# ddemidov/amgcl

Hardware: AMD Instinct MI355X
Metric: setup+solve time (s) & iterations to 1e-6, 3D Poisson 512^3 (lower is better)
Workload: dtype fp64; 1 GPU; model=3D Poisson 512^3 (7-point stencil), unknowns=134217728, solver=cg, precond=smoothed_aggregation AMG + SPAI0, iters=16, parallelism=single GPU

## Files before the change

amgcl_amd/backend/_hiplib.py:

```python
import ctypes
import os

_LIB = None

_SIGS = {
    "amg_spmv_f64": [ctypes.c_int64, ctypes.c_int64, ctypes.c_void_p, ctypes.c_void_p,
                     ctypes.c_void_p, ctypes.c_void_p, ctypes.c_double, ctypes.c_double,
                     ctypes.c_void_p, ctypes.c_int, ctypes.c_void_p],
    "amg_residual_f64": [ctypes.c_int64, ctypes.c_int64, ctypes.c_void_p, ctypes.c_void_p,
                         ctypes.c_void_p, ctypes.c_void_p, ctypes.c_void_p, ctypes.c_void_p,
                         ctypes.c_int, ctypes.c_void_p],
    "amg_relax_diag_f64": [ctypes.c_int64, ctypes.c_int64, ctypes.c_void_p, ctypes.c_void_p,
                           ctypes.c_void_p, ctypes.c_void_p, ctypes.c_void_p, ctypes.c_void_p,
                           ctypes.c_void_p, ctypes.c_int, ctypes.c_void_p],
    "amg_axpby_f64": [ctypes.c_int64, ctypes.c_double, ctypes.c_void_p, ctypes.c_double,
                      ctypes.c_void_p, ctypes.c_void_p],
    "amg_axpbypcz_f64": [ctypes.c_int64, ctypes.c_double, ctypes.c_void_p, ctypes.c_double,
                         ctypes.c_void_p, ctypes.c_double, ctypes.c_void_p, ctypes.c_void_p],
    "amg_vmul_f64": [ctypes.c_int64, ctypes.c_double, ctypes.c_void_p, ctypes.c_void_p,
                     ctypes.c_double, ctypes.c_void_p, ctypes.c_void_p],
    "amg_fill_f64": [ctypes.c_int64, ctypes.c_double, ctypes.c_void_p, ctypes.c_void_p],
    "amg_dot_f64": [ctypes.c_int64, ctypes.c_void_p, ctypes.c_void_p, ctypes.c_void_p,
                    ctypes.c_void_p],
    "amg_dot2_f64": [ctypes.c_int64, ctypes.c_void_p, ctypes.c_void_p, ctypes.c_void_p,
# ... 72 lines not shown
    "amg_sort_rows": [ctypes.c_int64] + [ctypes.c_void_p] * 4,
    "amg_spgemm_count": [ctypes.c_int64] + [ctypes.c_void_p] * 9,
    "amg_spgemm_fill": [ctypes.c_int64] + [ctypes.c_void_p] * 10 + [ctypes.c_int]
                       + [ctypes.c_void_p] * 2,
    "amg_gershgorin": [ctypes.c_int64, ctypes.c_void_p, ctypes.c_void_p, ctypes.c_void_p, ctypes.c_int, ctypes.c_void_p, ctypes.c_void_p],
    "amg_poisson_cnt": [ctypes.c_int64] * 4 + [ctypes.c_void_p] * 2,
    "amg_poisson_fill": [ctypes.c_int64] * 4 + [ctypes.c_void_p] * 4,
}

for _op in ("spmv", "residual", "relax_diag", "axpby", "axpbypcz", "vmul", "fill", "dot",
            "gather", "scatter", "gemv", "sell_spmv", "sell_residual", "sell_relax",
            "sell_fill"):
    _SIGS[f"amg_{_op}_f32"] = _SIGS[f"amg_{_op}_f64"]


def lib():
    global _LIB
    if _LIB is None:
        path = os.path.join(os.path.dirname(os.path.dirname(os.path.abspath(__file__))),
                            "_hip", "libamghip.so")
        if not os.path.exists(path):
            from ..build import build_hip_lib

            build_hip_lib()
        if not os.path.exists(path):
            raise RuntimeError(
                f"libamghip.so not found at {path}; run `python setup.py build_ext "
                "--inplace` — GPU ops do not fall back to eager torch"
            )
        _LIB = ctypes.CDLL(path)
        for name, argtypes in _SIGS.items():
            fn = getattr(_LIB, name)
            fn.argtypes = argtypes
            fn.restype = ctypes.c_int
    return _LIB


def check(rc, what):
    if rc != 0:
        raise RuntimeError(f"HIP kernel '{what}' failed with hipError_t={rc}")
```

amgcl_amd/csrc/hip/amg_common.h:

```cpp
#pragma once
#include <hip/hip_runtime.h>
#include <cstdint>

#define WAVE 64

__device__ static inline int64_t amg_logical_block() {
#ifdef AMGCL_SWIZZLE
    unsigned g = gridDim.x;
    if ((g & 7u) == 0u)
        return (int64_t)(blockIdx.x & 7u) * (int64_t)(g >> 3) + (blockIdx.x >> 3);
#endif
    return blockIdx.x;
}

#ifdef AMGCL_NT
#define AMG_STREAM_LD(p) __builtin_nontemporal_load(p)
#else
#define AMG_STREAM_LD(p) (*(p))
#endif

static inline int amg_nblocks(int64_t work, int block = 256, int cap = 2048) {
    int64_t b = (work + block - 1) / block;
    if (b < 1) b = 1;
    if (b > cap) b = cap;
    if (b > 8) b = (b + 7) & ~(int64_t)7;
    return (int)b;
}

static inline int amg_pick_subw(int64_t nrows, int64_t nnz) {
    double m = nrows ? (double)nnz / (double)nrows : 1.0;
    if (m <= 4) return 2;
    if (m <= 10) return 4;
    if (m <= 24) return 8;
    if (m <= 128) return 16;
// ... 45 lines not shown
```

amgcl_amd/csrc/hip/amg_kernels.h:

```cpp
#pragma once
#include <hip/hip_runtime.h>
#include <cstdint>

struct OpDesc;
struct LevelDesc;

extern "C" {

int amg_spmv_f64(int64_t nrows, int64_t nnz, const int *ptr, const int *col,
                 const double *val, const double *x, double alpha, double beta,
                 double *y, int subw, hipStream_t stream);
int amg_spmv_f32(int64_t nrows, int64_t nnz, const int *ptr, const int *col,
                 const float *val, const float *x, double alpha, double beta, float *y,
                 int subw, hipStream_t stream);
int amg_residual_f64(int64_t nrows, int64_t nnz, const int *ptr, const int *col,
                     const double *val, const double *rhs, const double *x, double *r,
                     int subw, hipStream_t stream);
int amg_residual_f32(int64_t nrows, int64_t nnz, const int *ptr, const int *col,
                     const float *val, const float *rhs, const float *x, float *r,
                     int subw, hipStream_t stream);
int amg_sell_spmv_f64(int64_t nrows, int64_t nslice, const int64_t *soff, const int *col,
                      const double *val, const int *srows, const double *x, double alpha,
                      double beta, double *y, hipStream_t stream);
int amg_sell_spmv_f32(int64_t nrows, int64_t nslice, const int64_t *soff, const int *col,
// ... 26 lines not shown
int amg_vmul_f64(int64_t n, double a, const double *m, const double *x, double b,
                 double *z, hipStream_t stream);
int amg_vmul_f32(int64_t n, double a, const float *m, const float *x, double b, float *z,
                 hipStream_t stream);
int amg_fill_f64(int64_t n, double v, double *x, hipStream_t stream);
int amg_fill_f32(int64_t n, double v, float *x, hipStream_t stream);
int amg_dot_f64(int64_t n, const double *x, const double *y, double *out,
                hipStream_t stream);
int amg_dot2_f64(int64_t n, const double *x1, const double *y1, const double *x2,
                 const double *y2, double *out, hipStream_t stream);
int amg_gemv_f64(int64_t n, const double *a, const double *f, double *u,
                 hipStream_t stream);
int amg_gemv_f32(int64_t n, const float *a, const float *f, float *u, hipStream_t stream);
int amg_cg_tail_f64(int64_t n, double alpha, const double *p, const double *q, double *x,
                    double *r, double *out, hipStream_t stream);
int amg_cast_d2s(int64_t n, const double *src, float *dst, hipStream_t stream);
int amg_cast_s2d(int64_t n, const float *src, double *dst, hipStream_t stream);

int amg_bsr_spmv_f64(int64_t nbrows, int bsize, const int *ptr, const int *col,
                     const double *val, const double *x, double alpha, double beta,
                     double *y, hipStream_t stream);
int amg_bsr_residual_f64(int64_t nbrows, int bsize, const int *ptr, const int *col,
                         const double *val, const double *rhs, const double *x,
                         double *r, hipStream_t stream);
int amg_bsr_relax_f64(int64_t nbrows, int bsize, const int *ptr, const int *col,
                      const double *val, const double *M, const double *rhs,
                      const double *x, double *t, hipStream_t stream);

int amg_setup_diag(int64_t n, const int *ptr, const int *col, const double *val,
                   double *d, hipStream_t s);
// ... 16 lines not shown
int amg_transpose_count(int64_t nnz, const int *col, int *tcnt, hipStream_t s);
int amg_transpose_scatter(int64_t n, const int *ptr, const int *col, const double *val,
                          int *cursor, int *tcol, double *tval, hipStream_t s);
int amg_spgemm_count(int64_t an, const int *aptr, const int *acol, const int *bptr,
                     const int *bcol, int *ub, int *cnt, int *overflow, int *bigscratch,
                     hipStream_t s);
int amg_spgemm_fill(int64_t an, const int *aptr, const int *acol, const double *aval,
                    const int *bptr, const int *bcol, const double *bval, const int *ub,
                    const int *cptr_scanned, int *ccol, double *cval, int do_sort,
                    const int *bigscratch, hipStream_t s);

void *amg_driver_create(const LevelDesc *levels, int nlevels, const void *coarse_inv,
                        int64_t ncoarse, int npre, int npost, int ncycle, int pre_cycles,
                        int f32, const OpDesc *a64, hipStream_t stream);
void amg_driver_destroy(void *h);
int amg_driver_precond(void *h, const double *rhs, double *x, double *x_swap);
int amg_driver_cg(void *h, const double *rhs, double *x, double *r, double *s, double *p,
                  double *q, double *s_swap, double tol, double abstol, int maxiter,
                  int64_t *iters_out, double *resid_out);
int amg_driver_bicgstab(void *h, const double *rhs, double *x, double *r, double *p,
                        double *v, double *s2, double *t2, double *rh, double *T,
                        double *T_swap, double tol, double abstol, int maxiter,
                        int64_t *iters_out, double *resid_out);

}
```

amgcl_amd/csrc/hip/driver.hip:

```cpp

#include <hip/hip_runtime.h>

#include "amg_common.h"
#include "amg_kernels.h"

#include <cmath>
#include <cstddef>
#include <cstdint>
#include <cstdlib>
#include <type_traits>
#include <utility>
#include <vector>

#define AMG_BY_TYPE(name)                                 \
    template <typename T, typename... Args>               \
    static inline int name(Args... args) {                \
        if constexpr (std::is_same_v<T, double>)          \
            return amg_##name##_f64(args...);             \
        else                                              \
            return amg_##name##_f32(args...);             \
    }
AMG_BY_TYPE(spmv)
AMG_BY_TYPE(residual)
AMG_BY_TYPE(gemv)
AMG_BY_TYPE(sell_spmv)
AMG_BY_TYPE(sell_residual)
AMG_BY_TYPE(sell_relax)
AMG_BY_TYPE(axpby)
AMG_BY_TYPE(vmul)
AMG_BY_TYPE(fill)
#undef AMG_BY_TYPE

template <int SUBW, typename T>
__global__ void relax_swap_k(int64_t nrows, const int *__restrict__ ptr,
                             const int *__restrict__ col, const T *__restrict__ val,
                             const T *__restrict__ M, const T *__restrict__ rhs,
                             const T *__restrict__ x, T *__restrict__ xn) {
    int64_t tid = amg_logical_block() * blockDim.x + threadIdx.x;
    int lane = (int)(tid & (SUBW - 1));
    int64_t row = tid / SUBW;
    int64_t stride = ((int64_t)gridDim.x * blockDim.x) / SUBW;
    for (; row < nrows; row += stride) {
        T s = (T)0;
        int b = ptr[row], e = ptr[row + 1];
        for (int j = b + lane; j < e; j += SUBW)
            s += AMG_STREAM_LD(&val[j]) * x[AMG_STREAM_LD(&col[j])];
#pragma unroll
        for (int off = SUBW / 2; off > 0; off >>= 1) s += __shfl_down(s, off, SUBW);
        if (lane == 0) xn[row] = x[row] + M[row] * (rhs[row] - s);
    }
}

template <typename T>
__global__ void relax_zero_k(int64_t n, const T *__restrict__ M,
                             const T *__restrict__ rhs, T *__restrict__ xn) {
    int64_t i = (int64_t)blockIdx.x * blockDim.x + threadIdx.x;
    int64_t stride = (int64_t)gridDim.x * blockDim.x;
    for (; i < n; i += stride) xn[i] = M[i] * rhs[i];
}

struct GraphEntry {
    const double *rhs;
    double *x;
    double *xswap;
    hipGraphExec_t exec;
};

struct Driver {
    std::vector<LevelDesc> lv;
    const void *coarse_inv;
    int64_t ncoarse;
    int npre, npost, ncycle, pre_cycles;
    hipStream_t stream;
    double *dotbuf_d;
    double *dotbuf_h;
    std::vector<GraphEntry> graphs;
    bool use_graphs;
    hipStream_t ext_stream;
    hipEvent_t ev_in, ev_out;
    int f32;
    OpDesc a64;
    float *cb_r, *cb_x, *cb_s;
};

#define CHK(x)                          \
    do {                                \
        int _rc = (x);                  \
        if (_rc) return _rc;            \
    } while (0)

template <typename T>
static int op_spmv(Driver *D, const OpDesc &op, const T *x, double alpha, double beta,
                   T *y) {
    if (op.nslice)
        return sell_spmv<T>(op.nrows, op.nslice, op.soff, op.scol, (const T *)op.sval,
                            op.srows, x, alpha, beta, y, D->stream);
    return spmv<T>(op.nrows, op.nnz, op.ptr, op.col, (const T *)op.val, x, alpha, beta, y,
                   op.subw, D->stream);
// ... 57 lines not shown
        CHK(amg_axpby_f64(n, 1.0, t, 1.0, s, st));
        CHK(amg_axpby_f64(n, om, s, 1.0 - om, y, st));
    }
    CHK(hipMemcpyAsync(b, y, n * sizeof(double), hipMemcpyDeviceToDevice, st));
    CHK(amg_vmul_f64(n, 1.0, L.ilu_dinv, b, 0.0, y, st));
    for (int it = 0; it < L.ilu_iters; ++it) {
        CHK(op_spmv<double>(D, L.ilu_U, y, -1.0, 0.0, s));
        CHK(amg_axpby_f64(n, 1.0, b, 1.0, s, st));
        CHK(amg_vmul_f64(n, 1.0, L.ilu_dinv, s, 0.0, s, st));
        CHK(amg_axpby_f64(n, om, s, 1.0 - om, y, st));
    }
    CHK(amg_axpby_f64(n, L.ilu_damping, y, 1.0, x, st));
    return 0;
}

template <typename T>
static int relax_swap(Driver *D, const LevelDesc &L, const T *rhs, T **x, T **xn) {
    if (L.ilu_iters) {
        CHK(ilu_apply<T>(D, L, rhs, *x, *xn));
        return 0;
    }
    if (L.cheb_degree) {
        CHK(cheb_apply<T>(D, L, rhs, *x, *xn));
        return 0;
    }
    if (L.bsize) {
        if constexpr (std::is_same_v<T, double>)
            CHK(amg_bsr_relax_f64(L.nbrows, L.bsize, L.bptr, L.bcol, L.bval, L.M, rhs,
                                  *x, *xn, D->stream));
        else
            return (int)hipErrorInvalidValue;
        CHK(axpby<T>(L.A.nrows, 1.0, *x, 1.0, *xn, D->stream));
        std::swap(*x, *xn);
        return 0;
    }
    const OpDesc &A = L.A;
    const T *M = (const T *)L.M;
    if (A.nslice) {
        CHK(sell_relax<T>(A.nrows, A.nslice, A.soff, A.scol, (const T *)A.sval, A.srows,
                          M, rhs, *x, *xn, D->stream));
        std::swap(*x, *xn);
        return 0;
    }
    int grid = amg_nblocks(A.nrows * A.subw);
    const T *val = (const T *)A.val;
#define RCASE(SW)                                                                       \
    case SW:                                                                            \
        relax_swap_k<SW, T><<<grid, 256, 0, D->stream>>>(A.nrows, A.ptr, A.col, val, M, \
                                                         rhs, *x, *xn);                 \
        break;
    switch (A.subw) {
        RCASE(1) RCASE(2) RCASE(4) RCASE(8) RCASE(16) RCASE(32) RCASE(64)
        default: return hipErrorInvalidValue;
    }
#undef RCASE
    std::swap(*x, *xn);
    return (int)hipGetLastError();
}

template <typename T>
static int cycle(Driver *D, int li, const T *f, T **u_io, T **scratch, bool u_is_zero) {
    LevelDesc &L = D->lv[li];
    const bool coarsest = (li + 1 == (int)D->lv.size());

    auto relax_zero = [&](LevelDesc &LL, const T *ff, T **u2, T **sc) -> int {
        if (LL.cheb_degree || LL.bsize || LL.ilu_iters) {
            CHK(fill<T>(LL.A.nrows, 0.0, *u2, D->stream));
            return relax_swap<T>(D, LL, ff, u2, sc);
        }
        relax_zero_k<T><<<amg_nblocks(LL.A.nrows), 256, 0, D->stream>>>(
            LL.A.nrows, (const T *)LL.M, ff, *sc);
        std::swap(*u2, *sc);
        return 0;
    };

    if (coarsest) {
        if (D->coarse_inv) {
            CHK(gemv<T>(L.A.nrows, (const T *)D->coarse_inv, f, *u_io, D->stream));
        } else {
            for (int i = 0; i < D->npre + D->npost; ++i) {
                if (u_is_zero && i == 0) {
                    CHK(relax_zero(L, f, u_io, scratch));
                    continue;
                }
                CHK(relax_swap<T>(D, L, f, u_io, scratch));
            }
// ... 6 lines not shown
        if (u_is_zero && i == 0) {
            CHK(relax_zero(L, f, u_io, scratch));
            continue;
        }
        CHK(relax_swap<T>(D, L, f, u_io, scratch));
    }
    CHK(level_residual<T>(D, L, f, *u_io, *scratch));
    CHK(op_spmv<T>(D, L.R, *scratch, 1.0, 0.0, (T *)N.f));
    T *nu = (T *)N.u;
    T *nscratch = (T *)N.t;
    for (int c = 0; c < D->ncycle; ++c) {
        CHK(cycle<T>(D, li + 1, (const T *)N.f, &nu, &nscratch, c == 0));
    }
    CHK(op_spmv<T>(D, L.P, nu, 1.0, 1.0, *u_io));
    for (int i = 0; i < D->npost; ++i)
        CHK(relax_swap<T>(D, L, f, u_io, scratch));
    return (int)hipGetLastError();
}

static int precond_apply(Driver *D, const double *rhs, double *x, double *x_swap) {
    const int64_t n = D->lv[0].A.nrows;
    if (D->f32) {
        CHK(amg_cast_d2s(n, rhs, D->cb_r, D->stream));
        float *u = D->cb_x;
        float *scratch = D->cb_s;
        for (int c = 0; c < D->pre_cycles; ++c)
            CHK(cycle<float>(D, 0, D->cb_r, &u, &scratch, c == 0));
        CHK(amg_cast_s2d(n, u, x, D->stream));
        return 0;
    }
    double *u = x;
    double *scratch = x_swap;
    for (int c = 0; c < D->pre_cycles; ++c)
        CHK(cycle<double>(D, 0, rhs, &u, &scratch, c == 0));
    if (u != x)
        CHK(hipMemcpyAsync(x, u, n * sizeof(double), hipMemcpyDeviceToDevice, D->stream));
    return 0;
}

static int precond_apply_graphed(Driver *D, const double *rhs, double *x,
                                 double *x_swap) {
    if (!D->use_graphs) return precond_apply(D, rhs, x, x_swap);
    for (const GraphEntry &g : D->graphs)
        if (g.rhs == rhs && g.x == x && g.xswap == x_swap)
            return (int)hipGraphLaunch(g.exec, D->stream);
    if (D->graphs.size() >= 8) return precond_apply(D, rhs, x, x_swap);
    if (hipStreamBeginCapture(D->stream, hipStreamCaptureModeThreadLocal) !=
        hipSuccess)
        return precond_apply(D, rhs, x, x_swap);
    int rc = precond_apply(D, rhs, x, x_swap);
    hipGraph_t graph;
    hipError_t ec = hipStreamEndCapture(D->stream, &graph);
    if (rc) return rc;
    if (ec != hipSuccess) return (int)ec;
    hipGraphExec_t exec;
    ec = hipGraphInstantiate(&exec, graph, nullptr, nullptr, 0);
    (void)hipGraphDestroy(graph);
    if (ec != hipSuccess) {
        (void)hipGetLastError();
        D->use_graphs = false;
        return precond_apply(D, rhs, x, x_swap);
    }
    D->graphs.push_back({rhs, x, x_swap, exec});
    return (int)hipGraphLaunch(exec, D->stream);
}

static int enter_driver(Driver *D) {
    if (D->stream == D->ext_stream) return 0;
    CHK((int)hipEventRecord(D->ev_in, D->ext_stream));
    CHK((int)hipStreamWaitEvent(D->stream, D->ev_in, 0));
    return 0;
}
static int leave_driver(Driver *D) {
    if (D->stream == D->ext_stream) return 0;
    CHK((int)hipEventRecord(D->ev_out, D->stream));
    CHK((int)hipStreamWaitEvent(D->ext_stream, D->ev_out, 0));
    return 0;
}

static int read_dots(Driver *D, int n, double *out) {
    CHK(hipMemcpyAsync(D->dotbuf_h, D->dotbuf_d, n * sizeof(double),
                       hipMemcpyDeviceToHost, D->stream));
    CHK(hipStreamSynchronize(D->stream));
    for (int i = 0; i < n; ++i) out[i] = D->dotbuf_h[i];
    return 0;
}

extern "C" void *amg_driver_create(const LevelDesc *levels, int nlevels,
                                   const void *coarse_inv, int64_t ncoarse, int npre,
                                   int npost, int ncycle, int pre_cycles, int f32,
                                   const OpDesc *a64, hipStream_t stream) {
    if (f32 && !a64) return nullptr;
    Driver *D = new Driver();
    D->lv.assign(levels, levels + nlevels);
    if (a64) D->a64 = *a64;
    auto settle = [](OpDesc &op) {
// ... 1 lines not shown
    };
    settle(D->a64);
    for (LevelDesc &L : D->lv)
        for (OpDesc *op : {&L.A, &L.P, &L.R, &L.ilu_L, &L.ilu_U}) settle(*op);
    D->coarse_inv = coarse_inv;
    D->ncoarse = ncoarse;
    D->npre = npre;
    D->npost = npost;
    D->ncycle = ncycle;
    D->pre_cycles = pre_cycles;
    D->stream = stream;
    D->f32 = f32;
    D->cb_r = D->cb_x = D->cb_s = nullptr;
    const char *ng = getenv("AMGCL_NO_GRAPH");
    D->use_graphs = !(ng && ng[0] && ng[0] != '0');
    D->ext_stream = stream;
    D->ev_in = D->ev_out = nullptr;
    hipStream_t st_int = nullptr;
    if (hipStreamCreateWithFlags(&st_int, hipStreamNonBlocking) == hipSuccess &&
        hipEventCreateWithFlags(&D->ev_in, hipEventDisableTiming) == hipSuccess &&
        hipEventCreateWithFlags(&D->ev_out, hipEventDisableTiming) == hipSuccess) {
        D->stream = st_int;
    } else {
        if (st_int) (void)hipStreamDestroy(st_int);
        D->use_graphs = false;
    }
    bool ok = hipMalloc((void **)&D->dotbuf_d, 2 * sizeof(double)) == hipSuccess &&
              hipHostMalloc((void **)&D->dotbuf_h, 2 * sizeof(double)) == hipSuccess;
    if (ok && f32) {
        int64_t n = D->lv[0].A.nrows;
        ok = hipMalloc((void **)&D->cb_r, n * sizeof(float)) == hipSuccess &&
             hipMalloc((void **)&D->cb_x, n * sizeof(float)) == hipSuccess &&
             hipMalloc((void **)&D->cb_s, n * sizeof(float)) == hipSuccess;
    }
    if (!ok) {
        delete D;
        return nullptr;
    }
    return D;
}

extern "C" void amg_driver_destroy(void *h) {
    Driver *D = (Driver *)h;
// ... 40 lines not shown
    return finish(D, precond_apply_graphed(D, rhs, x, x_swap), false);
}

struct FineOp {
    Driver *D;
    OpDesc op;
    const LevelDesc *bsr;
    explicit FineOp(Driver *D)
        : D(D), op(D->f32 ? D->a64 : D->lv[0].A),
          bsr(!D->f32 && D->lv[0].bsize ? &D->lv[0] : nullptr) {}
    int spmv(const double *x, double alpha, double beta, double *y) const {
        if (bsr)
            return amg_bsr_spmv_f64(bsr->nbrows, bsr->bsize, bsr->bptr, bsr->bcol,
                                    bsr->bval, x, alpha, beta, y, D->stream);
        return op_spmv<double>(D, op, x, alpha, beta, y);
    }
    int residual(const double *rhs, const double *x, double *r) const {
        return bsr ? level_residual<double>(D, *bsr, rhs, x, r)
                   : op_residual<double>(D, op, rhs, x, r);
    }
};

struct Krylov {
    double norm_rhs, eps, res;
};

static int krylov_begin(Driver *D, const FineOp &A, const double *rhs, double *x,
                        double *r, double *r_copy, double tol, double abstol,
                        Krylov *k) {
    const int64_t n = A.op.nrows;
// ... 19 lines not shown
    *iters_out = iter;
    *resid_out = k.norm_rhs == 0.0 ? 0.0 : k.res / k.norm_rhs;
    return 0;
}

static int cg_solve(Driver *D, const double *rhs, double *x, double *r, double *s,
                    double *p, double *q, double *s_swap, double tol, double abstol,
                    int maxiter, int64_t *iters_out, double *resid_out) {
    const FineOp A(D);
    const int64_t n = A.op.nrows;
    hipStream_t st = D->stream;
    double dots[2];
    Krylov k;
    CHK(krylov_begin(D, A, rhs, x, r, nullptr, tol, abstol, &k));

    double rho1 = 0.0, rho2 = 0.0;
    int64_t iter = 0;
    while (k.res > k.eps && iter < maxiter) {
        CHK(precond_apply_graphed(D, r, s, s_swap));
        rho2 = rho1;
        CHK(amg_dot_f64(n, r, s, D->dotbuf_d, st));
        CHK(read_dots(D, 1, dots));
        rho1 = dots[0];
        if (iter == 0) {
            CHK(hipMemcpyAsync(p, s, n * sizeof(double), hipMemcpyDeviceToDevice, st));
        } else {
            CHK(amg_axpby_f64(n, 1.0, s, rho1 / rho2, p, st));
        }
        CHK(A.spmv(p, 1.0, 0.0, q));
        CHK(amg_dot_f64(n, q, p, D->dotbuf_d, st));
        CHK(read_dots(D, 1, dots));
        double alpha = rho1 / dots[0];
        CHK(amg_cg_tail_f64(n, alpha, p, q, x, r, D->dotbuf_d, st));
        CHK(read_dots(D, 1, dots));
        k.res = sqrt(dots[0]);
        ++iter;
    }
    return krylov_end(k, iter, iters_out, resid_out);
}

extern "C" int amg_driver_cg(void *h, const double *rhs, double *x, double *r, double *s,
                             double *p, double *q, double *s_swap, double tol,
                             double abstol, int maxiter, int64_t *iters_out,
                             double *resid_out) {
    Driver *D = (Driver *)h;
    CHK(enter_driver(D));
    return finish(D, cg_solve(D, rhs, x, r, s, p, q, s_swap, tol, abstol, maxiter,
                              iters_out, resid_out), true);
}
// ... 68 lines not shown
```

amgcl_amd/csrc/hip/kernels.hip:

```cpp

#include <hip/hip_runtime.h>

#include <cstdint>
#include <cstdio>
#include <type_traits>

#include "amg_common.h"
#include "amg_kernels.h"


extern "C" int amg_hip_last_error() { return (int)hipGetLastError(); }

template <typename T, int SUBW, bool BETA0>
__global__ void spmv_k(int nrows, const int *__restrict__ ptr,
                       const int *__restrict__ col, const T *__restrict__ val,
                       const T *__restrict__ x, double alpha, double beta,
                       T *__restrict__ y) {
    int64_t tid = amg_logical_block() * blockDim.x + threadIdx.x;
    int lane = (int)(tid & (SUBW - 1));
    int64_t row = tid / SUBW;
    int64_t stride = ((int64_t)gridDim.x * blockDim.x) / SUBW;
    for (; row < nrows; row += stride) {
        double s = 0.0;
        int b = ptr[row], e = ptr[row + 1];
        for (int j = b + lane; j < e; j += SUBW) s += (double)AMG_STREAM_LD(&val[j]) * (double)x[AMG_STREAM_LD(&col[j])];
#pragma unroll
        for (int off = SUBW / 2; off > 0; off >>= 1) s += __shfl_down(s, off, SUBW);
        if (lane == 0) y[row] = (T)(BETA0 ? alpha * s : alpha * s + beta * (double)y[row]);
    }
}

template <typename T, int SUBW>
__global__ void residual_k(int nrows, const int *__restrict__ ptr,
                           const int *__restrict__ col, const T *__restrict__ val,
                           const T *__restrict__ rhs, const T *__restrict__ x,
                           T *__restrict__ r) {
    int64_t tid = amg_logical_block() * blockDim.x + threadIdx.x;
    int lane = (int)(tid & (SUBW - 1));
    int64_t row = tid / SUBW;
    int64_t stride = ((int64_t)gridDim.x * blockDim.x) / SUBW;
    for (; row < nrows; row += stride) {
        double s = 0.0;
        int b = ptr[row], e = ptr[row + 1];
        for (int j = b + lane; j < e; j += SUBW) s += (double)AMG_STREAM_LD(&val[j]) * (double)x[AMG_STREAM_LD(&col[j])];
// ... 25 lines not shown
template <typename F>
static int by_subw(int subw, int64_t nrows, int64_t nnz, F launch) {
    if (subw <= 0) subw = amg_pick_subw(nrows, nnz);
#define CASE(SW)                                     \
    case SW:                                         \
        launch(std::integral_constant<int, SW>{});   \
        break;
    switch (subw) {
        CASE(1) CASE(2) CASE(4) CASE(8) CASE(16) CASE(32) CASE(64)
        default: return (int)hipErrorInvalidValue;
    }
#undef CASE
    return (int)hipGetLastError();
}

template <typename T>
static int launch_spmv(int64_t nrows, int64_t nnz, const int *ptr, const int *col,
                       const T *val, const T *x, double alpha, double beta, T *y,
                       int subw, hipStream_t stream) {
    return by_subw(subw, nrows, nnz, [&](auto sw) {
        constexpr int SW = decltype(sw)::value;
        const int grid = amg_nblocks(nrows * SW);
        if (beta == 0.0)
            spmv_k<T, SW, true><<<grid, 256, 0, stream>>>(nrows, ptr, col, val, x, alpha, beta, y);
        else
            spmv_k<T, SW, false><<<grid, 256, 0, stream>>>(nrows, ptr, col, val, x, alpha, beta, y);
    });
}

template <typename T>
static int launch_residual(int64_t nrows, int64_t nnz, const int *ptr, const int *col,
                           const T *val, const T *rhs, const T *x, T *r, int subw,
                           hipStream_t stream) {
    return by_subw(subw, nrows, nnz, [&](auto sw) {
        constexpr int SW = decltype(sw)::value;
        residual_k<T, SW><<<amg_nblocks(nrows * SW), 256, 0, stream>>>(nrows, ptr, col, val,
                                                                      rhs, x, r);
    });
}

template <typename T>
// ... 5 lines not shown
        relax_diag_k<T, SW><<<amg_nblocks(nrows * SW), 256, 0, stream>>>(nrows, ptr, col,
                                                                        val, M, rhs, x, t);
    });
}

extern "C" int amg_spmv_f64(int64_t nrows, int64_t nnz, const int *ptr, const int *col,
                            const double *val, const double *x, double alpha,
                            double beta, double *y, int subw, hipStream_t stream) {
    return launch_spmv(nrows, nnz, ptr, col, val, x, alpha, beta, y, subw, stream);
}
extern "C" int amg_spmv_f32(int64_t nrows, int64_t nnz, const int *ptr, const int *col,
                            const float *val, const float *x, double alpha, double beta,
                            float *y, int subw, hipStream_t stream) {
    return launch_spmv(nrows, nnz, ptr, col, val, x, alpha, beta, y, subw, stream);
}

extern "C" int amg_residual_f64(int64_t nrows, int64_t nnz, const int *ptr, const int *col,
                                const double *val, const double *rhs, const double *x,
                                double *r, int subw, hipStream_t stream) {
    return launch_residual(nrows, nnz, ptr, col, val, rhs, x, r, subw, stream);
}
extern "C" int amg_residual_f32(int64_t nrows, int64_t nnz, const int *ptr, const int *col,
                                const float *val, const float *rhs, const float *x,
                                float *r, int subw, hipStream_t stream) {
    return launch_residual(nrows, nnz, ptr, col, val, rhs, x, r, subw, stream);
}

extern "C" int amg_relax_diag_f64(int64_t nrows, int64_t nnz, const int *ptr,
                                  const int *col, const double *val, const double *M,
                                  const double *rhs, const double *x, double *t,
                                  int subw, hipStream_t stream) {
    return launch_relax_diag(nrows, nnz, ptr, col, val, M, rhs, x, t, subw, stream);
}
extern "C" int amg_relax_diag_f32(int64_t nrows, int64_t nnz, const int *ptr,
                                  const int *col, const float *val, const float *M,
                                  const float *rhs, const float *x, float *t, int subw,
                                  hipStream_t stream) {
    return launch_relax_diag(nrows, nnz, ptr, col, val, M, rhs, x, t, subw, stream);
}

template <typename T, int MODE>
__global__ void sell_k(int64_t nrows, int64_t nslice,
                       const int64_t *__restrict__ soff, const int *__restrict__ col,
                       const T *__restrict__ val, const int *__restrict__ srows,
                       const T *__restrict__ x,
                       double alpha, double beta, const T *__restrict__ rhs,
                       const T *__restrict__ M, T *__restrict__ y) {
    const int wpb = blockDim.x / WAVE;
    int wid = threadIdx.x / WAVE, lane = threadIdx.x & (WAVE - 1);
    int64_t s = (int64_t)blockIdx.x * wpb + wid;
    int64_t sstride = (int64_t)gridDim.x * wpb;
    for (; s < nslice; s += sstride) {
        int64_t beg = soff[s], end = soff[s + 1];
        double acc = 0.0;
        for (int64_t j = beg + lane; j < end; j += WAVE)
            acc += (double)val[j] * (double)x[col[j]];
        int64_t row = srows ? (int64_t)srows[s * WAVE + lane] : s * WAVE + lane;
        if (row >= 0 && row < nrows) {
            if (MODE == 0)
                y[row] = (T)(beta == 0.0 ? alpha * acc
                                         : alpha * acc + beta * (double)y[row]);
            else if (MODE == 1)
                y[row] = (T)((double)rhs[row] - acc);
            else
                y[row] = (T)((double)x[row] +
                             (double)M[row] * ((double)rhs[row] - acc));
        }
    }
}

template <typename T, int MODE>
static int launch_sell(int64_t nrows, int64_t nslice, const int64_t *soff, const int *col,
                       const T *val, const int *srows, const T *x, double alpha,
                       double beta, const T *rhs, const T *M, T *y, hipStream_t stream) {
    sell_k<T, MODE><<<amg_nblocks(nslice * WAVE), 256, 0, stream>>>(
        nrows, nslice, soff, col, val, srows, x, alpha, beta, rhs, M, y);
    return (int)hipGetLastError();
}

extern "C" int amg_sell_spmv_f64(int64_t nrows, int64_t nslice, const int64_t *soff,
                                 const int *col, const double *val, const int *srows,
                                 const double *x, double alpha, double beta, double *y,
                                 hipStream_t stream) {
    return launch_sell<double, 0>(nrows, nslice, soff, col, val, srows, x, alpha, beta,
                                  nullptr, nullptr, y, stream);
}
extern "C" int amg_sell_spmv_f32(int64_t nrows, int64_t nslice, const int64_t *soff,
                                 const int *col, const float *val, const int *srows,
                                 const float *x, double alpha, double beta, float *y,
                                 hipStream_t stream) {
    return launch_sell<float, 0>(nrows, nslice, soff, col, val, srows, x, alpha, beta,
                                 nullptr, nullptr, y, stream);
}

extern "C" int amg_sell_residual_f64(int64_t nrows, int64_t nslice, const int64_t *soff,
                                     const int *col, const double *val, const int *srows,
                                     const double *rhs, const double *x, double *r,
                                     hipStream_t stream) {
    return launch_sell<double, 1>(nrows, nslice, soff, col, val, srows, x, 0.0, 0.0, rhs,
                                  nullptr, r, stream);
}
extern "C" int amg_sell_residual_f32(int64_t nrows, int64_t nslice, const int64_t *soff,
                                     const int *col, const float *val, const int *srows,
                                     const float *rhs, const float *x, float *r,
                                     hipStream_t stream) {
    return launch_sell<float, 1>(nrows, nslice, soff, col, val, srows, x, 0.0, 0.0, rhs,
                                 nullptr, r, stream);
}

extern "C" int amg_sell_relax_f64(int64_t nrows, int64_t nslice, const int64_t *soff,
                                  const int *col, const double *val, const int *srows,
                                  const double *M, const double *rhs, const double *x,
                                  double *xn, hipStream_t stream) {
    return launch_sell<double, 2>(nrows, nslice, soff, col, val, srows, x, 0.0, 0.0, rhs,
                                  M, xn, stream);
}
extern "C" int amg_sell_relax_f32(int64_t nrows, int64_t nslice, const int64_t *soff,
                                  const int *col, const float *val, const int *srows,
                                  const float *M, const float *rhs, const float *x,
                                  float *xn, hipStream_t stream) {
    return launch_sell<float, 2>(nrows, nslice, soff, col, val, srows, x, 0.0, 0.0, rhs,
                                 M, xn, stream);
}

template <typename T>
__global__ void sell_fill_k(int64_t nrows, int64_t nslice, const int *__restrict__ ptr,
                            const int *__restrict__ col, const T *__restrict__ val,
                            const int64_t *__restrict__ soff,
                            const int *__restrict__ srows, int *__restrict__ scol,
                            T *__restrict__ sval) {
// ... 397 lines not shown
            if (c == i) d = v;
            else s -= v * x[c];
        }
        x[i] = s / d;
    }
}

extern "C" int amg_gs_color_f64(int64_t nlist, const int *rows, const int *ptr,
                                const int *col, const double *val, const double *b,
                                double *x, hipStream_t stream) {
    gs_color_k<<<amg_nblocks(nlist), 256, 0, stream>>>(nlist, rows, ptr, col, val, b, x);
    return (int)hipGetLastError();
}


__global__ void cg_tail_k(int64_t n, double alpha, const double *__restrict__ p,
                          const double *__restrict__ q, double *__restrict__ x,
                          double *__restrict__ r, double *__restrict__ out) {
    __shared__ double lds[4];
    int64_t i = (int64_t)blockIdx.x * blockDim.x + threadIdx.x;
    int64_t stride = (int64_t)gridDim.x * blockDim.x;
    double s = 0.0;
    for (; i < n; i += stride) {
        x[i] += alpha * p[i];
        double rn = r[i] - alpha * q[i];
        r[i] = rn;
        s += rn * rn;
    }
#pragma unroll
    for (int off = WAVE / 2; off > 0; off >>= 1) s += __shfl_down(s, off, WAVE);
    int wid = threadIdx.x / WAVE, lane = threadIdx.x & (WAVE - 1);
    if (lane == 0) lds[wid] = s;
    __syncthreads();
    if (threadIdx.x == 0) atomicAdd(out, lds[0] + lds[1] + lds[2] + lds[3]);
}

extern "C" int amg_cg_tail_f64(int64_t n, double alpha, const double *p, const double *q,
                               double *x, double *r, double *out, hipStream_t stream) {
    fill_k<double><<<1, 64, 0, stream>>>(1, 0.0, out);
    cg_tail_k<<<amg_nblocks(n, 256, 2048), 256, 0, stream>>>(n, alpha, p, q, x, r, out);
    return (int)hipGetLastError();
}

struct c128 {
    double re, im;
};
__device__ static inline c128 cmul(c128 a, c128 b) {
    return {a.re * b.re - a.im * b.im, a.re * b.im + a.im * b.re};
}
__device__ static inline c128 cmulc(c128 a, c128 b) {
    return {a.re * b.re + a.im * b.im, a.re * b.im - a.im * b.re};
}
__device__ static inline c128 cadd(c128 a, c128 b) { return {a.re + b.re, a.im + b.im}; }
__device__ static inline c128 csub(c128 a, c128 b) { return {a.re - b.re, a.im - b.im}; }

// ... 175 lines not shown
```

Baseline: 834.5 ms.

## Fuse CG dot products into SpMV, relaxation and tail kernels

Adds dot-product epilogues to the SpMV, SELL relax and CSR relax kernels so that the CG inner products (p·q, r·s) come out of the kernels that already produce those vectors. Accumulator zeroing is moved into earlier kernels instead of separate fill launches. This removes extra vector-read passes and small kernel launches per iteration on a bandwidth-bound solve. In exchange it adds atomics and an LDS reduction to those kernels, plus more bookkeeping and more variants of captured graphs.

Result: faster. 826.2 ms (median of 6 runs) (-1.0%).

```diff
diff --git a/amgcl_amd/backend/_hiplib.py b/amgcl_amd/backend/_hiplib.py
--- a/amgcl_amd/backend/_hiplib.py
+++ b/amgcl_amd/backend/_hiplib.py
@@ -110,6 +110,16 @@
     _SIGS[f"amg_{_op}_f32"] = _SIGS[f"amg_{_op}_f64"]
 
 
+_FUSED_SIGS = {
+    "amg_spmv_dot_f64": [ctypes.c_int64, ctypes.c_int64] + [ctypes.c_void_p] * 7
+                        + [ctypes.c_int, ctypes.c_void_p],
+    "amg_sell_spmv_dot_f64": [ctypes.c_int64, ctypes.c_int64] + [ctypes.c_void_p] * 9,
+    "amg_sell_relax_dot_f64": [ctypes.c_int64, ctypes.c_int64] + [ctypes.c_void_p] * 10,
+    "amg_relax_swap_f64": [ctypes.c_int64, ctypes.c_int64] + [ctypes.c_void_p] * 8
+                          + [ctypes.c_int, ctypes.c_void_p],
+}
+
+
 def lib():
     global _LIB
     if _LIB is None:
@@ -125,7 +135,7 @@
                 "--inplace` — GPU ops do not fall back to eager torch"
             )
         _LIB = ctypes.CDLL(path)
-        for name, argtypes in _SIGS.items():
+        for name, argtypes in {**_SIGS, **_FUSED_SIGS}.items():
             fn = getattr(_LIB, name)
             fn.argtypes = argtypes
             fn.restype = ctypes.c_int
diff --git a/amgcl_amd/csrc/hip/amg_common.h b/amgcl_amd/csrc/hip/amg_common.h
--- a/amgcl_amd/csrc/hip/amg_common.h
+++ b/amgcl_amd/csrc/hip/amg_common.h
@@ -18,6 +18,24 @@
 #else
 #define AMG_STREAM_LD(p) (*(p))
 #endif
+
+struct DotOut {
+    double *out;
+    double *zero;
+};
+
+__device__ static inline void amg_dot_epilogue(double s, DotOut d) {
+    __shared__ double lds[4];
+#pragma unroll
+    for (int off = WAVE / 2; off > 0; off >>= 1) s += __shfl_down(s, off, WAVE);
+    int wid = threadIdx.x / WAVE, lane = threadIdx.x & (WAVE - 1);
+    if (lane == 0) lds[wid] = s;
+    __syncthreads();
+    if (threadIdx.x == 0) {
+        atomicAdd(d.out, lds[0] + lds[1] + lds[2] + lds[3]);
+        if (d.zero && blockIdx.x == 0) *d.zero = 0.0;
+    }
+}
 
 static inline int amg_nblocks(int64_t work, int block = 256, int cap = 2048) {
     int64_t b = (work + block - 1) / block;
diff --git a/amgcl_amd/csrc/hip/amg_kernels.h b/amgcl_amd/csrc/hip/amg_kernels.h
--- a/amgcl_amd/csrc/hip/amg_kernels.h
+++ b/amgcl_amd/csrc/hip/amg_kernels.h
@@ -64,6 +64,20 @@
 int amg_gemv_f32(int64_t n, const float *a, const float *f, float *u, hipStream_t stream);
 int amg_cg_tail_f64(int64_t n, double alpha, const double *p, const double *q, double *x,
                     double *r, double *out, hipStream_t stream);
+int amg_spmv_dot_f64(int64_t nrows, int64_t nnz, const int *ptr, const int *col,
+                     const double *val, const double *x, double *y, double *out,
+                     double *zero, int subw, hipStream_t stream);
+int amg_sell_spmv_dot_f64(int64_t nrows, int64_t nslice, const int64_t *soff,
+                          const int *col, const double *val, const int *srows,
+                          const double *x, double *y, double *out, double *zero,
+                          hipStream_t stream);
+int amg_sell_relax_dot_f64(int64_t nrows, int64_t nslice, const int64_t *soff,
+                           const int *col, const double *val, const int *srows,
+                           const double *M, const double *rhs, const double *x,
+                           double *xn, double *out, hipStream_t stream);
+int amg_cg_tail_nofill_f64(int64_t n, double alpha, const double *p, const double *q,
+                           double *x, double *r, double *out, double *zero,
+                           hipStream_t stream);
 int amg_cast_d2s(int64_t n, const double *src, float *dst, hipStream_t stream);
 int amg_cast_s2d(int64_t n, const float *src, double *dst, hipStream_t stream);
 
@@ -110,6 +124,10 @@
                         int64_t ncoarse, int npre, int npost, int ncycle, int pre_cycles,
                         int f32, const OpDesc *a64, hipStream_t stream);
 void amg_driver_destroy(void *h);
+int amg_relax_swap_f64(int64_t nrows, int64_t nnz, const int *ptr, const int *col,
+                       const double *val, const double *M, const double *rhs,
+                       const double *x, double *xn, double *out, int subw,
+                       hipStream_t stream);
 int amg_driver_precond(void *h, const double *rhs, double *x, double *x_swap);
 int amg_driver_cg(void *h, const double *rhs, double *x, double *r, double *s, double *p,
                   double *q, double *s_swap, double tol, double abstol, int maxiter,
diff --git a/amgcl_amd/csrc/hip/driver.hip b/amgcl_amd/csrc/hip/driver.hip
--- a/amgcl_amd/csrc/hip/driver.hip
+++ b/amgcl_amd/csrc/hip/driver.hip
@@ -31,15 +31,16 @@
 AMG_BY_TYPE(fill)
 #undef AMG_BY_TYPE
 
-template <int SUBW, typename T>
+template <int SUBW, typename T, typename... Dot>
 __global__ void relax_swap_k(int64_t nrows, const int *__restrict__ ptr,
                              const int *__restrict__ col, const T *__restrict__ val,
                              const T *__restrict__ M, const T *__restrict__ rhs,
-                             const T *__restrict__ x, T *__restrict__ xn) {
+                             const T *__restrict__ x, T *__restrict__ xn, Dot... dot) {
     int64_t tid = amg_logical_block() * blockDim.x + threadIdx.x;
     int lane = (int)(tid & (SUBW - 1));
     int64_t row = tid / SUBW;
     int64_t stride = ((int64_t)gridDim.x * blockDim.x) / SUBW;
+    [[maybe_unused]] double prod = 0.0;
     for (; row < nrows; row += stride) {
         T s = (T)0;
         int b = ptr[row], e = ptr[row + 1];
@@ -47,15 +48,26 @@
             s += AMG_STREAM_LD(&val[j]) * x[AMG_STREAM_LD(&col[j])];
 #pragma unroll
         for (int off = SUBW / 2; off > 0; off >>= 1) s += __shfl_down(s, off, SUBW);
-        if (lane == 0) xn[row] = x[row] + M[row] * (rhs[row] - s);
-    }
-}
-
-template <typename T>
+        if constexpr (sizeof...(Dot) == 0) {
+            if (lane == 0) xn[row] = x[row] + M[row] * (rhs[row] - s);
+        } else if (lane == 0) {
+            T f = rhs[row];
+            T v = x[row] + M[row] * (f - s);
+            xn[row] = v;
+            prod += (double)f * (double)v;
+        }
+    }
+    if constexpr (sizeof...(Dot) != 0) amg_dot_epilogue(prod, (dot, ...));
+}
+
+template <typename T, typename... Zero>
 __global__ void relax_zero_k(int64_t n, const T *__restrict__ M,
-                             const T *__restrict__ rhs, T *__restrict__ xn) {
+                             const T *__restrict__ rhs, T *__restrict__ xn,
+                             Zero... zero) {
     int64_t i = (int64_t)blockIdx.x * blockDim.x + threadIdx.x;
     int64_t stride = (int64_t)gridDim.x * blockDim.x;
+    if constexpr (sizeof...(Zero) != 0)
+        if (i == 0) *(zero, ...) = 0.0;
     for (; i < n; i += stride) xn[i] = M[i] * rhs[i];
 }
 
@@ -63,6 +75,7 @@
     const double *rhs;
     double *x;
     double *xswap;
+    double *dot;
     hipGraphExec_t exec;
 };
 
@@ -74,6 +87,7 @@
     hipStream_t stream;
     double *dotbuf_d;
     double *dotbuf_h;
+    bool fuse_dots;
     std::vector<GraphEntry> graphs;
     bool use_graphs;
     hipStream_t ext_stream;
@@ -82,6 +96,8 @@
     OpDesc a64;
     float *cb_r, *cb_x, *cb_s;
 };
+
+enum { NDOTS = 4 };
 
 #define CHK(x)                          \
     do {                                \
@@ -169,8 +185,45 @@
     return 0;
 }
 
+template <typename T, typename... Dot>
+static int launch_relax_swap(const OpDesc &A, const T *M, const T *rhs, const T *x,
+                             T *xn, hipStream_t stream, Dot... dot) {
+    int grid = amg_nblocks(A.nrows * A.subw);
+    const T *val = (const T *)A.val;
+#define RCASE(SW)                                                                      \
+    case SW:                                                                           \
+        relax_swap_k<SW, T, Dot...><<<grid, 256, 0, stream>>>(A.nrows, A.ptr, A.col,   \
+                                                              val, M, rhs, x, xn,      \
+                                                              dot...);                 \
+        break;
+    switch (A.subw) {
+        RCASE(1) RCASE(2) RCASE(4) RCASE(8) RCASE(16) RCASE(32) RCASE(64)
+        default: return hipErrorInvalidValue;
+    }
+#undef RCASE
+    return (int)hipGetLastError();
+}
+
+extern "C" int amg_relax_swap_f64(int64_t nrows, int64_t nnz, const int *ptr,
+                                  const int *col, const double *val, const double *M,
+                                  const double *rhs, const double *x, double *xn,
+                                  double *out, int subw, hipStream_t stream) {
+    OpDesc A{};
+    A.nrows = nrows, A.nnz = nnz, A.ptr = ptr, A.col = col, A.val = val;
+    A.subw = subw > 0 ? subw : amg_pick_subw(nrows, nnz);
+    return out ? launch_relax_swap(A, M, rhs, x, xn, stream, DotOut{out, nullptr})
+               : launch_relax_swap(A, M, rhs, x, xn, stream);
+}
+
+static bool plain_relax(const LevelDesc &L) {
+    return !L.ilu_iters && !L.cheb_degree && !L.bsize;
+}
+
 template <typename T>
-static int relax_swap(Driver *D, const LevelDesc &L, const T *rhs, T **x, T **xn) {
+static int relax_swap(Driver *D, const LevelDesc &L, const T *rhs, T **x, T **xn,
+                      double *dot = nullptr) {
+    if (dot && !(plain_relax(L) && std::is_same_v<T, double>))
+        return (int)hipErrorInvalidValue;
     if (L.ilu_iters) {
         CHK(ilu_apply<T>(D, L, rhs, *x, *xn));
         return 0;
@@ -191,40 +244,45 @@
     }
     const OpDesc &A = L.A;
     const T *M = (const T *)L.M;
-    if (A.nslice) {
+    if constexpr (std::is_same_v<T, double>) {
+        if (dot) {
+            if (A.nslice)
+                CHK(amg_sell_relax_dot_f64(A.nrows, A.nslice, A.soff, A.scol,
+                                           (const double *)A.sval, A.srows, M, rhs, *x,
+                                           *xn, dot, D->stream));
+            else
+                CHK(launch_relax_swap(A, M, rhs, *x, *xn, D->stream,
+                                      DotOut{dot, nullptr}));
+            std::swap(*x, *xn);
+            return 0;
+        }
+    }
+    if (A.nslice)
         CHK(sell_relax<T>(A.nrows, A.nslice, A.soff, A.scol, (const T *)A.sval, A.srows,
                           M, rhs, *x, *xn, D->stream));
-        std::swap(*x, *xn);
-        return 0;
-    }
-    int grid = amg_nblocks(A.nrows * A.subw);
-    const T *val = (const T *)A.val;
-#define RCASE(SW)                                                                       \
-    case SW:                                                                            \
-        relax_swap_k<SW, T><<<grid, 256, 0, D->stream>>>(A.nrows, A.ptr, A.col, val, M, \
-                                                         rhs, *x, *xn);                 \
-        break;
-    switch (A.subw) {
-        RCASE(1) RCASE(2) RCASE(4) RCASE(8) RCASE(16) RCASE(32) RCASE(64)
-        default: return hipErrorInvalidValue;
-    }
-#undef RCASE
+    else
+        CHK(launch_relax_swap(A, M, rhs, *x, *xn, D->stream));
     std::swap(*x, *xn);
-    return (int)hipGetLastError();
+    return 0;
 }
 
 template <typename T>
-static int cycle(Driver *D, int li, const T *f, T **u_io, T **scratch, bool u_is_zero) {
+static int cycle(Driver *D, int li, const T *f, T **u_io, T **scratch, bool u_is_zero,
+                 double *zero = nullptr, double *dot = nullptr) {
     LevelDesc &L = D->lv[li];
     const bool coarsest = (li + 1 == (int)D->lv.size());
 
     auto relax_zero = [&](LevelDesc &LL, const T *ff, T **u2, T **sc) -> int {
-        if (LL.cheb_degree || LL.bsize || LL.ilu_iters) {
+        if (!plain_relax(LL)) {
             CHK(fill<T>(LL.A.nrows, 0.0, *u2, D->stream));
             return relax_swap<T>(D, LL, ff, u2, sc);
         }
-        relax_zero_k<T><<<amg_nblocks(LL.A.nrows), 256, 0, D->stream>>>(
-            LL.A.nrows, (const T *)LL.M, ff, *sc);
+        if (zero)
+            relax_zero_k<T><<<amg_nblocks(LL.A.nrows), 256, 0, D->stream>>>(
+                LL.A.nrows, (const T *)LL.M, ff, *sc, zero);
+        else
+            relax_zero_k<T><<<amg_nblocks(LL.A.nrows), 256, 0, D->stream>>>(
+                LL.A.nrows, (const T *)LL.M, ff, *sc);
         std::swap(*u2, *sc);
         return 0;
     };
@@ -261,11 +319,20 @@
     }
     CHK(op_spmv<T>(D, L.P, nu, 1.0, 1.0, *u_io));
     for (int i = 0; i < D->npost; ++i)
-        CHK(relax_swap<T>(D, L, f, u_io, scratch));
+        CHK(relax_swap<T>(D, L, f, u_io, scratch, i + 1 == D->npost ? dot : nullptr));
     return (int)hipGetLastError();
 }
 
-static int precond_apply(Driver *D, const double *rhs, double *x, double *x_swap) {
+static bool fused_rs_ok(const Driver *D) {
+    return !D->f32 && D->npost >= 1 && D->pre_cycles >= 1 && D->lv.size() > 1 &&
+           plain_relax(D->lv[0]);
+}
+static bool zero_in_smooth(const Driver *D) {
+    return D->npre >= 1 && D->lv.size() > 1 && plain_relax(D->lv[0]);
+}
+
+static int precond_apply(Driver *D, const double *rhs, double *x, double *x_swap,
+                         double *dot = nullptr) {
     const int64_t n = D->lv[0].A.nrows;
     if (D->f32) {
         CHK(amg_cast_d2s(n, rhs, D->cb_r, D->stream));
@@ -278,24 +345,28 @@
     }
     double *u = x;
     double *scratch = x_swap;
+    if (dot && !fused_rs_ok(D)) return (int)hipErrorInvalidValue;
+    if (dot && !zero_in_smooth(D)) CHK(amg_fill_f64(1, 0.0, dot, D->stream));
     for (int c = 0; c < D->pre_cycles; ++c)
-        CHK(cycle<double>(D, 0, rhs, &u, &scratch, c == 0));
+        CHK(cycle<double>(D, 0, rhs, &u, &scratch, c == 0,
+                          c == 0 && zero_in_smooth(D) ? dot : nullptr,
+                          c + 1 == D->pre_cycles ? dot : nullptr));
     if (u != x)
         CHK(hipMemcpyAsync(x, u, n * sizeof(double), hipMemcpyDeviceToDevice, D->stream));
     return 0;
 }
 
 static int precond_apply_graphed(Driver *D, const double *rhs, double *x,
-                                 double *x_swap) {
-    if (!D->use_graphs) return precond_apply(D, rhs, x, x_swap);
+                                 double *x_swap, double *dot = nullptr) {
+    if (!D->use_graphs) return precond_apply(D, rhs, x, x_swap, dot);
     for (const GraphEntry &g : D->graphs)
-        if (g.rhs == rhs && g.x == x && g.xswap == x_swap)
+        if (g.rhs == rhs && g.x == x && g.xswap == x_swap && g.dot == dot)
             return (int)hipGraphLaunch(g.exec, D->stream);
-    if (D->graphs.size() >= 8) return precond_apply(D, rhs, x, x_swap);
+    if (D->graphs.size() >= 8) return precond_apply(D, rhs, x, x_swap, dot);
     if (hipStreamBeginCapture(D->stream, hipStreamCaptureModeThreadLocal) !=
         hipSuccess)
-        return precond_apply(D, rhs, x, x_swap);
-    int rc = precond_apply(D, rhs, x, x_swap);
+        return precond_apply(D, rhs, x, x_swap, dot);
+    int rc = precond_apply(D, rhs, x, x_swap, dot);
     hipGraph_t graph;
     hipError_t ec = hipStreamEndCapture(D->stream, &graph);
     if (rc) return rc;
@@ -306,9 +377,9 @@
     if (ec != hipSuccess) {
         (void)hipGetLastError();
         D->use_graphs = false;
-        return precond_apply(D, rhs, x, x_swap);
-    }
-    D->graphs.push_back({rhs, x, x_swap, exec});
+        return precond_apply(D, rhs, x, x_swap, dot);
+    }
+    D->graphs.push_back({rhs, x, x_swap, dot, exec});
     return (int)hipGraphLaunch(exec, D->stream);
 }
 
@@ -325,8 +396,8 @@
     return 0;
 }
 
-static int read_dots(Driver *D, int n, double *out) {
-    CHK(hipMemcpyAsync(D->dotbuf_h, D->dotbuf_d, n * sizeof(double),
+static int read_dots(Driver *D, int n, double *out, int first = 0) {
+    CHK(hipMemcpyAsync(D->dotbuf_h, D->dotbuf_d + first, n * sizeof(double),
                        hipMemcpyDeviceToHost, D->stream));
     CHK(hipStreamSynchronize(D->stream));
     for (int i = 0; i < n; ++i) out[i] = D->dotbuf_h[i];
@@ -358,6 +429,8 @@
     D->cb_r = D->cb_x = D->cb_s = nullptr;
     const char *ng = getenv("AMGCL_NO_GRAPH");
     D->use_graphs = !(ng && ng[0] && ng[0] != '0');
+    const char *nf = getenv("AMGCL_NO_FUSED_DOTS");
+    D->fuse_dots = !(nf && nf[0] && nf[0] != '0');
     D->ext_stream = stream;
     D->ev_in = D->ev_out = nullptr;
     hipStream_t st_int = nullptr;
@@ -369,8 +442,8 @@
         if (st_int) (void)hipStreamDestroy(st_int);
         D->use_graphs = false;
     }
-    bool ok = hipMalloc((void **)&D->dotbuf_d, 2 * sizeof(double)) == hipSuccess &&
-              hipHostMalloc((void **)&D->dotbuf_h, 2 * sizeof(double)) == hipSuccess;
+    bool ok = hipMalloc((void **)&D->dotbuf_d, NDOTS * sizeof(double)) == hipSuccess &&
+              hipHostMalloc((void **)&D->dotbuf_h, NDOTS * sizeof(double)) == hipSuccess;
     if (ok && f32) {
         int64_t n = D->lv[0].A.nrows;
         ok = hipMalloc((void **)&D->cb_r, n * sizeof(float)) == hipSuccess &&
@@ -441,6 +514,19 @@
             return amg_bsr_spmv_f64(bsr->nbrows, bsr->bsize, bsr->bptr, bsr->bcol,
                                     bsr->bval, x, alpha, beta, y, D->stream);
         return op_spmv<double>(D, op, x, alpha, beta, y);
+    }
+    int spmv_dot(const double *x, double *y, double *out, double *zero) const {
+        if (bsr) {
+            CHK(spmv(x, 1.0, 0.0, y));
+            CHK(amg_dot_f64(op.nrows, y, x, out, D->stream));
+            return amg_fill_f64(1, 0.0, zero, D->stream);
+        }
+        if (op.nslice)
+            return amg_sell_spmv_dot_f64(op.nrows, op.nslice, op.soff, op.scol,
+                                         (const double *)op.sval, op.srows, x, y, out,
+                                         zero, D->stream);
+        return amg_spmv_dot_f64(op.nrows, op.nnz, op.ptr, op.col, (const double *)op.val,
+                                x, y, out, zero, op.subw, D->stream);
     }
     int residual(const double *rhs, const double *x, double *r) const {
         return bsr ? level_residual<double>(D, *bsr, rhs, x, r)
@@ -490,25 +576,38 @@
     Krylov k;
     CHK(krylov_begin(D, A, rhs, x, r, nullptr, tol, abstol, &k));
 
+    enum { RS = 0, QP = 1, RR = 2 };
+    double *const slot = D->dotbuf_d;
+    const bool fuse = D->fuse_dots;
+    const bool fuse_rs = fuse && fused_rs_ok(D);
+    if (fuse) CHK(amg_fill_f64(1, 0.0, slot + QP, st));
+
     double rho1 = 0.0, rho2 = 0.0;
     int64_t iter = 0;
     while (k.res > k.eps && iter < maxiter) {
-        CHK(precond_apply_graphed(D, r, s, s_swap));
+        CHK(precond_apply_graphed(D, r, s, s_swap, fuse_rs ? slot + RS : nullptr));
         rho2 = rho1;
-        CHK(amg_dot_f64(n, r, s, D->dotbuf_d, st));
-        CHK(read_dots(D, 1, dots));
+        if (!fuse_rs) CHK(amg_dot_f64(n, r, s, slot + RS, st));
+        CHK(read_dots(D, 1, dots, RS));
         rho1 = dots[0];
         if (iter == 0) {
             CHK(hipMemcpyAsync(p, s, n * sizeof(double), hipMemcpyDeviceToDevice, st));
         } else {
             CHK(amg_axpby_f64(n, 1.0, s, rho1 / rho2, p, st));
         }
-        CHK(A.spmv(p, 1.0, 0.0, q));
-        CHK(amg_dot_f64(n, q, p, D->dotbuf_d, st));
-        CHK(read_dots(D, 1, dots));
+        if (fuse) {
+            CHK(A.spmv_dot(p, q, slot + QP, slot + RR));
+        } else {
+            CHK(A.spmv(p, 1.0, 0.0, q));
+            CHK(amg_dot_f64(n, q, p, slot + QP, st));
+        }
+        CHK(read_dots(D, 1, dots, QP));
         double alpha = rho1 / dots[0];
-        CHK(amg_cg_tail_f64(n, alpha, p, q, x, r, D->dotbuf_d, st));
-        CHK(read_dots(D, 1, dots));
+        if (fuse)
+            CHK(amg_cg_tail_nofill_f64(n, alpha, p, q, x, r, slot + RR, slot + QP, st));
+        else
+            CHK(amg_cg_tail_f64(n, alpha, p, q, x, r, slot + RR, st));
+        CHK(read_dots(D, 1, dots, RR));
         k.res = sqrt(dots[0]);
         ++iter;
     }
diff --git a/amgcl_amd/csrc/hip/kernels.hip b/amgcl_amd/csrc/hip/kernels.hip
--- a/amgcl_amd/csrc/hip/kernels.hip
+++ b/amgcl_amd/csrc/hip/kernels.hip
@@ -11,23 +11,29 @@
 
 extern "C" int amg_hip_last_error() { return (int)hipGetLastError(); }
 
-template <typename T, int SUBW, bool BETA0>
+template <typename T, int SUBW, bool BETA0, typename... Dot>
 __global__ void spmv_k(int nrows, const int *__restrict__ ptr,
                        const int *__restrict__ col, const T *__restrict__ val,
                        const T *__restrict__ x, double alpha, double beta,
-                       T *__restrict__ y) {
+                       T *__restrict__ y, Dot... dot) {
     int64_t tid = amg_logical_block() * blockDim.x + threadIdx.x;
     int lane = (int)(tid & (SUBW - 1));
     int64_t row = tid / SUBW;
     int64_t stride = ((int64_t)gridDim.x * blockDim.x) / SUBW;
+    [[maybe_unused]] double prod = 0.0;
     for (; row < nrows; row += stride) {
         double s = 0.0;
         int b = ptr[row], e = ptr[row + 1];
         for (int j = b + lane; j < e; j += SUBW) s += (double)AMG_STREAM_LD(&val[j]) * (double)x[AMG_STREAM_LD(&col[j])];
 #pragma unroll
         for (int off = SUBW / 2; off > 0; off >>= 1) s += __shfl_down(s, off, SUBW);
-        if (lane == 0) y[row] = (T)(BETA0 ? alpha * s : alpha * s + beta * (double)y[row]);
-    }
+        if (lane == 0) {
+            T yn = (T)(BETA0 ? alpha * s : alpha * s + beta * (double)y[row]);
+            y[row] = yn;
+            if constexpr (sizeof...(Dot) != 0) prod += (double)x[row] * (double)yn;
+        }
+    }
+    if constexpr (sizeof...(Dot) != 0) amg_dot_epilogue(prod, (dot, ...));
 }
 
 template <typename T, int SUBW>
@@ -83,17 +89,21 @@
     return (int)hipGetLastError();
 }
 
-template <typename T>
+template <typename T, typename... Dot>
 static int launch_spmv(int64_t nrows, int64_t nnz, const int *ptr, const int *col,
                        const T *val, const T *x, double alpha, double beta, T *y,
-                       int subw, hipStream_t stream) {
+                       int subw, hipStream_t stream, Dot... dot) {
     return by_subw(subw, nrows, nnz, [&](auto sw) {
         constexpr int SW = decltype(sw)::value;
         const int grid = amg_nblocks(nrows * SW);
-        if (beta == 0.0)
-            spmv_k<T, SW, true><<<grid, 256, 0, stream>>>(nrows, ptr, col, val, x, alpha, beta, y);
-        else
-            spmv_k<T, SW, false><<<grid, 256, 0, stream>>>(nrows, ptr, col, val, x, alpha, beta, y);
+        if constexpr (sizeof...(Dot) == 0) {
+            if (beta == 0.0)
+                spmv_k<T, SW, true><<<grid, 256, 0, stream>>>(nrows, ptr, col, val, x, alpha, beta, y);
+            else
+                spmv_k<T, SW, false><<<grid, 256, 0, stream>>>(nrows, ptr, col, val, x, alpha, beta, y);
+        } else {
+            spmv_k<T, SW, true><<<grid, 256, 0, stream>>>(nrows, ptr, col, val, x, alpha, 0.0, y, dot...);
+        }
     });
 }
 
@@ -129,6 +139,13 @@
                             float *y, int subw, hipStream_t stream) {
     return launch_spmv(nrows, nnz, ptr, col, val, x, alpha, beta, y, subw, stream);
 }
+extern "C" int amg_spmv_dot_f64(int64_t nrows, int64_t nnz, const int *ptr, const int *col,
+                                const double *val, const double *x, double *y,
+                                double *out, double *zero, int subw,
+                                hipStream_t stream) {
+    return launch_spmv(nrows, nnz, ptr, col, val, x, 1.0, 0.0, y, subw, stream,
+                       DotOut{out, zero});
+}
 
 extern "C" int amg_residual_f64(int64_t nrows, int64_t nnz, const int *ptr, const int *col,
                                 const double *val, const double *rhs, const double *x,
@@ -154,17 +171,18 @@
     return launch_relax_diag(nrows, nnz, ptr, col, val, M, rhs, x, t, subw, stream);
 }
 
-template <typename T, int MODE>
+template <typename T, int MODE, typename... Dot>
 __global__ void sell_k(int64_t nrows, int64_t nslice,
                        const int64_t *__restrict__ soff, const int *__restrict__ col,
                        const T *__restrict__ val, const int *__restrict__ srows,
                        const T *__restrict__ x,
                        double alpha, double beta, const T *__restrict__ rhs,
-                       const T *__restrict__ M, T *__restrict__ y) {
+                       const T *__restrict__ M, T *__restrict__ y, Dot... dot) {
     const int wpb = blockDim.x / WAVE;
     int wid = threadIdx.x / WAVE, lane = threadIdx.x & (WAVE - 1);
     int64_t s = (int64_t)blockIdx.x * wpb + wid;
     int64_t sstride = (int64_t)gridDim.x * wpb;
+    [[maybe_unused]] double prod = 0.0;
     for (; s < nslice; s += sstride) {
         int64_t beg = soff[s], end = soff[s + 1];
         double acc = 0.0;
@@ -172,24 +190,39 @@
             acc += (double)val[j] * (double)x[col[j]];
         int64_t row = srows ? (int64_t)srows[s * WAVE + lane] : s * WAVE + lane;
         if (row >= 0 && row < nrows) {
-            if (MODE == 0)
-                y[row] = (T)(beta == 0.0 ? alpha * acc
-                                         : alpha * acc + beta * (double)y[row]);
-            else if (MODE == 1)
-                y[row] = (T)((double)rhs[row] - acc);
-            else
-                y[row] = (T)((double)x[row] +
-                             (double)M[row] * ((double)rhs[row] - acc));
-        }
-    }
-}
-
-template <typename T, int MODE>
+            if constexpr (sizeof...(Dot) == 0) {
+                if (MODE == 0)
+                    y[row] = (T)(beta == 0.0 ? alpha * acc
+                                             : alpha * acc + beta * (double)y[row]);
+                else if (MODE == 1)
+                    y[row] = (T)((double)rhs[row] - acc);
+                else
+                    y[row] = (T)((double)x[row] +
+                                 (double)M[row] * ((double)rhs[row] - acc));
+            } else if constexpr (MODE == 0) {
+                T yn = (T)(beta == 0.0 ? alpha * acc
+                                       : alpha * acc + beta * (double)y[row]);
+                y[row] = yn;
+                prod += (double)x[row] * (double)yn;
+            } else {
+                static_assert(MODE == 2, "no dot epilogue for the residual");
+                double f = (double)rhs[row];
+                T xn = (T)((double)x[row] + (double)M[row] * (f - acc));
+                y[row] = xn;
+                prod += f * (double)xn;
+            }
+        }
+    }
+    if constexpr (sizeof...(Dot) != 0) amg_dot_epilogue(prod, (dot, ...));
+}
+
+template <typename T, int MODE, typename... Dot>
 static int launch_sell(int64_t nrows, int64_t nslice, const int64_t *soff, const int *col,
                        const T *val, const int *srows, const T *x, double alpha,
-                       double beta, const T *rhs, const T *M, T *y, hipStream_t stream) {
-    sell_k<T, MODE><<<amg_nblocks(nslice * WAVE), 256, 0, stream>>>(
-        nrows, nslice, soff, col, val, srows, x, alpha, beta, rhs, M, y);
+                       double beta, const T *rhs, const T *M, T *y, hipStream_t stream,
+                       Dot... dot) {
+    sell_k<T, MODE, Dot...><<<amg_nblocks(nslice * WAVE), 256, 0, stream>>>(
+        nrows, nslice, soff, col, val, srows, x, alpha, beta, rhs, M, y, dot...);
     return (int)hipGetLastError();
 }
 
@@ -208,6 +241,14 @@
                                  nullptr, nullptr, y, stream);
 }
 
+extern "C" int amg_sell_spmv_dot_f64(int64_t nrows, int64_t nslice, const int64_t *soff,
+                                     const int *col, const double *val, const int *srows,
+                                     const double *x, double *y, double *out,
+                                     double *zero, hipStream_t stream) {
+    return launch_sell<double, 0>(nrows, nslice, soff, col, val, srows, x, 1.0, 0.0,
+                                  nullptr, nullptr, y, stream, DotOut{out, zero});
+}
+
 extern "C" int amg_sell_residual_f64(int64_t nrows, int64_t nslice, const int64_t *soff,
                                      const int *col, const double *val, const int *srows,
                                      const double *rhs, const double *x, double *r,
@@ -229,6 +270,13 @@
                                   double *xn, hipStream_t stream) {
     return launch_sell<double, 2>(nrows, nslice, soff, col, val, srows, x, 0.0, 0.0, rhs,
                                   M, xn, stream);
+}
+extern "C" int amg_sell_relax_dot_f64(int64_t nrows, int64_t nslice, const int64_t *soff,
+                                      const int *col, const double *val, const int *srows,
+                                      const double *M, const double *rhs, const double *x,
+                                      double *xn, double *out, hipStream_t stream) {
+    return launch_sell<double, 2>(nrows, nslice, soff, col, val, srows, x, 0.0, 0.0, rhs,
+                                  M, xn, stream, DotOut{out, nullptr});
 }
 extern "C" int amg_sell_relax_f32(int64_t nrows, int64_t nslice, const int64_t *soff,
                                   const int *col, const float *val, const int *srows,
@@ -656,9 +704,11 @@
 }
 
 
+template <typename... Zero>
 __global__ void cg_tail_k(int64_t n, double alpha, const double *__restrict__ p,
                           const double *__restrict__ q, double *__restrict__ x,
-                          double *__restrict__ r, double *__restrict__ out) {
+                          double *__restrict__ r, double *__restrict__ out,
+                          Zero... zero) {
     __shared__ double lds[4];
     int64_t i = (int64_t)blockIdx.x * blockDim.x + threadIdx.x;
     int64_t stride = (int64_t)gridDim.x * blockDim.x;
@@ -674,13 +724,24 @@
     int wid = threadIdx.x / WAVE, lane = threadIdx.x & (WAVE - 1);
     if (lane == 0) lds[wid] = s;
     __syncthreads();
-    if (threadIdx.x == 0) atomicAdd(out, lds[0] + lds[1] + lds[2] + lds[3]);
+    if (threadIdx.x == 0) {
+        atomicAdd(out, lds[0] + lds[1] + lds[2] + lds[3]);
+        if constexpr (sizeof...(Zero) != 0)
+            if (blockIdx.x == 0) *(zero, ...) = 0.0;
+    }
 }
 
 extern "C" int amg_cg_tail_f64(int64_t n, double alpha, const double *p, const double *q,
                                double *x, double *r, double *out, hipStream_t stream) {
     fill_k<double><<<1, 64, 0, stream>>>(1, 0.0, out);
     cg_tail_k<<<amg_nblocks(n, 256, 2048), 256, 0, stream>>>(n, alpha, p, q, x, r, out);
+    return (int)hipGetLastError();
+}
+extern "C" int amg_cg_tail_nofill_f64(int64_t n, double alpha, const double *p,
+                                      const double *q, double *x, double *r, double *out,
+                                      double *zero, hipStream_t stream) {
+    cg_tail_k<<<amg_nblocks(n, 256, 2048), 256, 0, stream>>>(n, alpha, p, q, x, r, out,
+                                                             zero);
     return (int)hipGetLastError();
 }
 
```
